# sebrahimi1988/dss-ml-at-scale

Measured on NVIDIA H100. Metric: series fitted+forecast/sec, higher is better.
Workload: dtype f32

## Files before the change

### dss-ml-at-scale_b200/csrc/fit_tc.cu

```cuda
#include "mmf_internal.cuh"
#include "sm90_ptx.cuh"

namespace mmf {
namespace {

using namespace sm90;

constexpr int TILE_M = 128;
constexpr int KC = 32;
constexpr int NGROUPS = 2;
constexpr int FOLD_CHUNKS = 18;
constexpr int MAX_PRED = 64;
constexpr int BULK_MAX_PRED = 28;
constexpr int Y_STAGE_BYTES = TILE_M * KC * 4;
constexpr int AT_STAGE_BYTES = 2 * P * KC * 4;
constexpr int THREADS = 416;
constexpr int TILE_RING = 4;
constexpr int WARP_EPI0 = 8, WARP_PROD = 12;

template <int STAGES, int OBUF, bool SE = false>
struct SmemLayoutT {
  static constexpr int y = 0;
  static constexpr int at = y + STAGES * Y_STAGE_BYTES;
  static constexpr int apred = at + STAGES * AT_STAGE_BYTES;
  static constexpr int ostage = apred + MAX_PRED * P * 4;
  static constexpr int acc = ostage + OBUF * TILE_M * BULK_MAX_PRED * 4;
  static constexpr int nm = acc + 2 * NGROUPS * TILE_M * P * 4;
  static constexpr int cc = nm + 2 * NGROUPS * TILE_M * 2;
  static constexpr int tiles = cc + 2 * TILE_M * 4;
  static constexpr int bars = tiles + TILE_RING * 4;
  static constexpr int n_bars = 2 * STAGES + 6 + 2 * TILE_RING;
  static constexpr int ss = bars + n_bars * 8;
  static constexpr int sfac = ss + (SE ? 2 * NGROUPS * TILE_M * 8 : 0);
  static constexpr int total = sfac + (SE ? MAX_PRED * 4 : 0);
  static_assert(total + 1024 <= 232448, "exceeds the 227 KB of shared memory a CTA can opt into");
};

__device__ __forceinline__ float dot16(const float* __restrict__ arow, const float (&g)[P], float s) {
  const float4* ap = reinterpret_cast<const float4*>(arow);
  const float4 a0 = ap[0], a1 = ap[1], a2 = ap[2], a3 = ap[3];
  s = fmaf(a0.x, g[0], s);  s = fmaf(a0.y, g[1], s);  s = fmaf(a0.z, g[2], s);  s = fmaf(a0.w, g[3], s);
  s = fmaf(a1.x, g[4], s);  s = fmaf(a1.y, g[5], s);  s = fmaf(a1.z, g[6], s);  s = fmaf(a1.w, g[7], s);
  s = fmaf(a2.x, g[8], s);  s = fmaf(a2.y, g[9], s);  s = fmaf(a2.z, g[10], s); s = fmaf(a2.w, g[11], s);
  s = fmaf(a3.x, g[12], s); s = fmaf(a3.y, g[13], s); s = fmaf(a3.z, g[14], s); s = fmaf(a3.w, g[15], s);
  return s;
}

__device__ __forceinline__ bool is_finite_bits(float x) { return (__float_as_uint(x) & 0x7f800000u) != 0x7f800000u; }

__device__ __forceinline__ float centring_constant(const float4& a, const float4& b, int t_fit) {
  const float v[8] = {a.x, a.y, a.z, a.w, b.x, b.y, b.z, b.w};
  float c = t_fit > 7 ? v[7] : __int_as_float(0x7fc00000);
#pragma unroll
  for (int i = 6; i >= 0; --i) c = (i < t_fit && is_finite_bits(v[i])) ? v[i] : c;
  return c;
}

__device__ __forceinline__ void bt_write_moments(const BtArgs& bt, int k, int grp, int64_t n, const TileRec& tr, int frow0,
                                                 int t4, const float (&acc)[2][P], bool folded, const float* sacc) {
#pragma unroll
  for (int h = 0; h < 2; ++h)
#pragma unroll
    for (int j = 0; j < 2; ++j) {
      const int rt = 64 * h + frow0 + 8 * j;
      if (rt >= tr.nrows) continue;
      float* __restrict__ dst = bt.mom + (((int64_t)k * 2 + grp) * n + tr.row0 + rt) * P + 2 * t4;
#pragma unroll
      for (int i = 0; i < 2; ++i) {
        const int q = 4 * i + 2 * j;
        float2 v = make_float2(acc[h][q] + acc[h][q + P / 2], acc[h][q + 1] + acc[h][q + 1 + P / 2]);
        if (folded) {
          const float2 o = *reinterpret_cast<const float2*>(sacc + rt * P + 8 * i + 2 * t4);
          v.x = o.x + v.x; v.y = o.y + v.y;
        }
        *reinterpret_cast<float2*>(dst + 8 * i) = v;
      }
    }
}

__device__ __forceinline__ float lds32(uint32_t addr) {
  float v;
  asm volatile("ld.shared.f32 %0, [%1];" : "=f"(v) : "r"(addr));
  return v;
}

template <int STAGES, int OBUF, bool MULTI, bool SE = false, bool BT = false>
__global__ void __launch_bounds__(THREADS, 1)
fit_tc_kernel(const __grid_constant__ TcLaunch tl, const DesignView d, const FitArgs a,
              uint32_t* __restrict__ pending_count, const int n_tiles, const int n_chunks, const MultiView mv,
              const SeArgs se, const BtArgs bt) {
  static_assert(!SE || !MULTI, "standard errors are built for the single-calendar launch");
  static_assert(!BT || !(MULTI || SE), "backtests are built for the single-calendar launch");
  using SmemLayout = SmemLayoutT<STAGES, OBUF, SE>;
  auto tile_rec = [&](int ti) -> TileRec {
    if (MULTI) {
      if (ti >= n_tiles) return TileRec{0, 0, 0, 1};
      const int4 v = __ldg(reinterpret_cast<const int4*>(mv.tiles) + ti);
      return TileRec{v.x, v.y, v.z, v.w};
    }
    const int64_t left = a.n - (int64_t)ti * TILE_M;
    return TileRec{ti * TILE_M, (int)(left >= TILE_M ? TILE_M : (left > 0 ? left : 0)), 0, n_chunks};
  };
  extern __shared__ unsigned char smem_dyn[];
  unsigned char* smem = reinterpret_cast<unsigned char*>((reinterpret_cast<uintptr_t>(smem_dyn) + 1023) & ~uintptr_t(1023));
  const uint32_t sbase = smem_u32(smem);
  const uint32_t s_y = sbase + SmemLayout::y;
  const uint32_t s_at = sbase + SmemLayout::at;
  float* s_apred = reinterpret_cast<float*>(smem + SmemLayout::apred);
  float* s_ostage = reinterpret_cast<float*>(smem + SmemLayout::ostage);
  float* s_acc = reinterpret_cast<float*>(smem + SmemLayout::acc);
  uint16_t* s_nm = reinterpret_cast<uint16_t*>(smem + SmemLayout::nm);
  float* s_cc = reinterpret_cast<float*>(smem + SmemLayout::cc);
  double* s_ss = reinterpret_cast<double*>(smem + SmemLayout::ss);
  float* s_sfac = reinterpret_cast<float*>(smem + SmemLayout::sfac);
#ifdef MMF_TC_NO_COLLECT
  const bool collect = false;
#else
  const bool collect = a.recs != nullptr && d.t_fit <= 65535;
#endif
  const uint32_t s_bars = sbase + SmemLayout::bars;
  const int warp = threadIdx.x >> 5;
  const int lane = threadIdx.x & 31;
  auto bar_full = [&](int s) { return s_bars + 8u * s; };
  auto bar_empty = [&](int s) { return s_bars + 8u * (STAGES + s); };
  auto bar_accfull = [&](int b) { return s_bars + 8u * (2 * STAGES + b); };
  auto bar_accempty = [&](int b) { return s_bars + 8u * (2 * STAGES + 2 + b); };
  auto bar_cc = [&](int b) { return s_bars + 8u * (2 * STAGES + 4 + b); };
  auto bar_tfull = [&](int s) { return s_bars + 8u * (2 * STAGES + 6 + s); };
  auto bar_tempty = [&](int s) { return s_bars + 8u * (2 * STAGES + 6 + TILE_RING + s); };
  int* s_tiles = reinterpret_cast<int*>(smem + SmemLayout::tiles);
  auto take_tile = [&](int lt) -> int {
    const int sl = lt % TILE_RING;
    mbar_wait(bar_tfull(sl), (lt / TILE_RING) & 1);
    const int t = *reinterpret_cast<volatile int*>(s_tiles + sl);
    __syncwarp();
    if (lane == 0) mbar_arrive(bar_tempty(sl));
    return t;
  };

  if (blockIdx.x == 0 && threadIdx.x == 0 && a.zero_next != nullptr) {
#pragma unroll
    for (int i = 0; i < CTR_WORDS; ++i) a.zero_next[i] = 0u;
  }
  if (warp == WARP_PROD) {
    if (lane == 0) {
      for (int s = 0; s < STAGES; ++s) {
        mbar_init(bar_full(s), 1);
        mbar_init(bar_empty(s), 4);
      }
      for (int b = 0; b < 2; ++b) {
        mbar_init(bar_accfull(b), NGROUPS * 128);
        mbar_init(bar_accempty(b), 4);
        mbar_init(bar_cc(b), 128);
      }
      for (int sl = 0; sl < TILE_RING; ++sl) {
        mbar_init(bar_tfull(sl), 1);
        mbar_init(bar_tempty(sl), NGROUPS * 4 + 4);
      }
      fence_mbar_init();
      prefetch_tensormap(tl.tmap_y);
      prefetch_tensormap(tl.tmap_at);
    }
  } else if (warp >= WARP_EPI0) {
    if (!a.skip_pred && !MULTI)
      for (int i = threadIdx.x - WARP_EPI0 * 32; i < a.n_pred * P; i += 128)
        s_apred[i] = __ldg(d.apred + (size_t)a.pred_start * P + i);
    if (SE && !a.skip_pred)
      for (int i = threadIdx.x - WARP_EPI0 * 32; i < a.n_pred; i += 128) s_sfac[i] = __ldg(se.sfac + a.pred_start + i);
  }
  __syncthreads();
  if (threadIdx.x == 0) pdl_launch_dependents();

  if (warp == WARP_PROD) {
    int stage = 0;
    uint32_t phase = 0;
    int last_cal = -1;
    uint32_t* claim_ctr = pending_count + CTR_TILE_CLAIM;
    int tile = blockIdx.x;
    for (int lt = 0;; ++lt) {
      const int sl = lt % TILE_RING;
      mbar_wait(bar_tempty(sl), ((lt / TILE_RING) & 1) ^ 1u);
      const bool more = tile < n_tiles;
      uint32_t claim = 0;
      if (lane == 0) {
        if (more) claim = atomicAdd(claim_ctr, 1u);
        s_tiles[sl] = more ? tile : -1;
        mbar_arrive(bar_tfull(sl));
      }
      __syncwarp();
      if (!more) break;
      const TileRec tr = tile_rec(tile);
      const void* tmy = MULTI ? static_cast<const void*>(mv.tmaps_y + (size_t)tr.cal * 128) : static_cast<const void*>(tl.tmap_y);
      if (MULTI && tr.cal != last_cal) { fence_tensormap_acquire(tmy); last_cal = tr.cal; }
      const int at_row = MULTI ? tr.cal * 2 * P : 0;
      for (int ch = 0; ch < tr.n_chunks; ++ch) {
        mbar_wait(bar_empty(stage), phase ^ 1u);
        tma_load_2d_x2_elect(bar_full(stage), Y_STAGE_BYTES + AT_STAGE_BYTES,
                             s_y + stage * Y_STAGE_BYTES, tmy, ch * KC, tr.row0, L2_EVICT_NORMAL,
                             s_at + stage * AT_STAGE_BYTES, tl.tmap_at, ch * KC, at_row,
                             MULTI ? L2_EVICT_NORMAL : L2_EVICT_LAST);
        if (++stage == STAGES) { stage = 0; phase ^= 1u; }
      }
      tile = static_cast<int>(gridDim.x + __shfl_sync(0xffffffffu, claim, 0));
    }
  } else if (warp < NGROUPS * 4) {
    const int grp = warp >> 2;
    const int r = threadIdx.x & 127;
    const uint32_t row_off = static_cast<uint32_t>(r) * 128u;
    const uint32_t sw = static_cast<uint32_t>(r & 7);
    const int g8 = lane >> 2, t4 = lane & 3;
    const int frow0 = 16 * (warp & 3) + g8;
    uint32_t gc = 0;
    for (int lt = 0;; ++lt) {
      const int tile = take_tile(lt);
      if (tile < 0) break;
      const TileRec tr = tile_rec(tile);
      bool bad = false;
      float cf[2][2];
      float acc[2][P];
#pragma unroll
      for (int h = 0; h < 2; ++h)
#pragma unroll
        for (int i = 0; i < P; ++i) acc[h][i] = 0.f;
      const bool scan = collect && (!MULTI || r < tr.nrows);
      const int seg = (grp ^ (int)gc) & 1;
      int nm = 0;
      unsigned long long packq = 0ull;
      const int ab = lt & 1;
      float* __restrict__ sacc = s_acc + (ab * NGROUPS + grp) * TILE_M * P;
      auto sacc_at = [&](int h, int j, int i) {
        return reinterpret_cast<float2*>(sacc + (64 * h + frow0 + 8 * j) * P + 8 * i + 2 * t4);
      };
      bool folded = false;
      int since_fold = 0;
      double ssq[2][2] = {{0.0, 0.0}, {0.0, 0.0}};
      for (int ch = seg; ch < tr.n_chunks; ch += NGROUPS) {
        const uint32_t k = gc + static_cast<uint32_t>(ch);
        const int stage = static_cast<int>(k % STAGES);
        mbar_wait(bar_full(stage), (k / STAGES) & 1u);
        const uint32_t sy = s_y + stage * Y_STAGE_BYTES;
        if (ch == seg) {
          if (seg == 0) {
            mbar_wait(bar_accempty(ab), ((lt >> 1) & 1) ^ 1u);
            float c = 0.f;
            if (d.has_constant && r < tr.nrows) {
              const uint32_t rowp = sy + row_off;
              c = centring_constant(lds128(rowp + (sw << 4)), lds128(rowp + ((1u ^ sw) << 4)), MULTI ? KC : d.t_fit);
            }
            bad = collect && !is_finite_bits(c);
            s_cc[ab * TILE_M + r] = bad ? 0.f : c;
            mbar_arrive(bar_cc(ab));
          }
          mbar_wait(bar_cc(ab), (lt >> 1) & 1);
#pragma unroll
          for (int h = 0; h < 2; ++h)
#pragma unroll
            for (int j = 0; j < 2; ++j) cf[h][j] = s_cc[ab * TILE_M + 64 * h + frow0 + 8 * j];
        }
        if (scan) {
          const uint32_t rowp = sy + row_off;
          float4 v[8];
#pragma unroll
          for (int q = 0; q < 8; ++q) v[q] = lds128(rowp + ((static_cast<uint32_t>(q) ^ sw) << 4));
          float chk = 0.f;
#pragma unroll
          for (int q = 0; q < 8; ++q) {
            chk = fmaf(v[q].x, 0.f, chk); chk = fmaf(v[q].y, 0.f, chk);
            chk = fmaf(v[q].z, 0.f, chk); chk = fmaf(v[q].w, 0.f, chk);
          }
          if (!(chk == 0.f)) {
            unsigned gaps = 0u;
#pragma unroll
            for (int q = 0; q < 8; ++q)
              gaps |= (is_finite_bits(v[q].x) ? 0u : 1u << (4 * q)) | (is_finite_bits(v[q].y) ? 0u : 2u << (4 * q)) |
                      (is_finite_bits(v[q].z) ? 0u : 4u << (4 * q)) | (is_finite_bits(v[q].w) ? 0u : 8u << (4 * q));
            uint16_t* __restrict__ mt = a.recs[(int64_t)tr.row0 + r].miss_t + seg * SOLVE_SEG;
            const int tbase = ch * KC;
            while (gaps) {
              const int pos = __ffs(gaps) - 1;
              gaps &= gaps - 1u;
              packq = (packq >> 16) | (static_cast<unsigned long long>(tbase + pos) << 48);
              ++nm;
              if ((nm & 3) == 0 && nm <= SOLVE_SEG) *reinterpret_cast<unsigned long long*>(mt + nm - 4) = packq;
              if constexpr (BT) if (nm == SOLVE_SEG + 1)
                reinterpret_cast<uint16_t*>(&a.recs[(int64_t)tr.row0 + r].ss)[seg] = static_cast<uint16_t>(tbase + pos);
            }
          }
        }
        uint32_t ahi[2][KC / 8][4], alo[2][KC / 8][4];
        const int lim = d.t_fit - ch * KC;
#pragma unroll
        for (int h = 0; h < 2; ++h)
#pragma unroll
          for (int j = 0; j < 2; ++j) {
            const uint32_t rowp = sy + static_cast<uint32_t>(64 * h + frow0 + 8 * j) * 128u + t4 * 4;
            float part = 0.f;
#pragma unroll
            for (int kk = 0; kk < KC / 8; ++kk)
#pragma unroll
              for (int hf = 0; hf < 2; ++hf) {
                float x = lds32(rowp + ((static_cast<uint32_t>(2 * kk + hf) ^ static_cast<uint32_t>(g8)) << 4));
                if (collect) x = is_finite_bits(x) ? x : cf[h][j];
                const float rr = x - cf[h][j];
                const uint32_t hb = __float_as_uint(rr) & 0xFFFFE000u;
                ahi[h][kk][j + 2 * hf] = hb;
                alo[h][kk][j + 2 * hf] = __float_as_uint(rr - __uint_as_float(hb));
                if (SE) {
                  const float rs = 4 * (2 * kk + hf) + t4 < lim ? rr : 0.f;
                  part = fmaf(rs, rs, part);
                }
              }
            if (SE) ssq[h][j] += static_cast<double>(part);
          }
        const uint64_t bdesc0 = gmma_desc_k_sw128(s_at + stage * AT_STAGE_BYTES);
        uint32_t bt_in = 0;
        if constexpr (BT) {
          const int s0 = ch * KC;
          uint32_t pre = 0;
#pragma unroll
          for (int k = 0; k < MMF_BT_MAX_ORIGINS - 1; ++k) {
            pre |= (bt.t_orig[k] >= s0 - KC && bt.t_orig[k] <= s0 ? 1u : 0u) << k;
            bt_in |= (bt.t_orig[k] > s0 && bt.t_orig[k] < s0 + KC ? 1u : 0u) << k;
          }
          while (pre) {
            const int k = __ffs(pre) - 1;
            pre &= pre - 1u;
            bt_write_moments(bt, k, grp, a.n, tr, frow0, t4, acc, folded, sacc);
          }
        }
        if constexpr (BT) {
        if (bt_in != 0u) {
          int lo = 0;
          uint32_t m = bt_in;
          for (;;) {
            const int k = m ? __ffs(m) - 1 : -1;
            const int hi = k >= 0 ? __ldg(&bt.cals[k].t_fit) - ch * KC : KC;
            wgmma_fence();
#pragma unroll
            for (int h = 0; h < 2; ++h)
#pragma unroll
              for (int kk = 0; kk < KC / 8; ++kk) {
                const uint64_t bdesc = bdesc0 + static_cast<uint64_t>(kk * 2);
                uint32_t fh[4], fl[4];
#pragma unroll
                for (int e = 0; e < 4; ++e) {
                  const int col = 8 * kk + 4 * (e >> 1) + t4;
                  const bool in = col >= lo && col < hi;
                  fh[e] = in ? ahi[h][kk][e] : 0u;
                  fl[e] = in ? alo[h][kk][e] : 0u;
                }
                wgmma_m64n32k8_tf32_rs(acc[h], fh, bdesc);
#ifndef MMF_TC_NO_LO_TERM
                wgmma_m64n32k8_tf32_rs(acc[h], fl, bdesc);
#endif
              }
            wgmma_commit();
            wgmma_wait<0>();
            wgmma_fence_regs(acc[0]);
            wgmma_fence_regs(acc[1]);
            if (k < 0) break;
            bt_write_moments(bt, k, grp, a.n, tr, frow0, t4, acc, folded, sacc);
            m &= m - 1u;
            lo = hi;
          }
        } else {
        wgmma_fence();
#pragma unroll
        for (int h = 0; h < 2; ++h)
#pragma unroll
          for (int kk = 0; kk < KC / 8; ++kk) {
            const uint64_t bdesc = bdesc0 + static_cast<uint64_t>(kk * 2);
            wgmma_m64n32k8_tf32_rs(acc[h], ahi[h][kk], bdesc);
#ifndef MMF_TC_NO_LO_TERM
            wgmma_m64n32k8_tf32_rs(acc[h], alo[h][kk], bdesc);
#endif
          }
        wgmma_commit();
        wgmma_wait<0>();
        wgmma_fence_regs(acc[0]);
        wgmma_fence_regs(acc[1]);
        }
        } else {
        wgmma_fence();
#pragma unroll
        for (int h = 0; h < 2; ++h)
#pragma unroll
          for (int kk = 0; kk < KC / 8; ++kk) {
            const uint64_t bdesc = bdesc0 + static_cast<uint64_t>(kk * 2);
            wgmma_m64n32k8_tf32_rs(acc[h], ahi[h][kk], bdesc);
#ifndef MMF_TC_NO_LO_TERM
            wgmma_m64n32k8_tf32_rs(acc[h], alo[h][kk], bdesc);
#endif
          }
        wgmma_commit();
        wgmma_wait<0>();
        wgmma_fence_regs(acc[0]);
        wgmma_fence_regs(acc[1]);
        }
        __syncwarp();
        if (lane == 0) mbar_arrive(bar_empty(stage));
        if (++since_fold == FOLD_CHUNKS && ch + NGROUPS < tr.n_chunks) {
          if (!folded) mbar_wait(bar_accempty(ab), ((lt >> 1) & 1) ^ 1u);
#pragma unroll
          for (int h = 0; h < 2; ++h)
#pragma unroll
            for (int j = 0; j < 2; ++j)
#pragma unroll
              for (int i = 0; i < 2; ++i) {
                const int q = 4 * i + 2 * j;
                float2 f = make_float2(acc[h][q] + acc[h][q + P / 2], acc[h][q + 1] + acc[h][q + 1 + P / 2]);
                if (folded) { const float2 o = *sacc_at(h, j, i); f.x = o.x + f.x; f.y = o.y + f.y; }
                *sacc_at(h, j, i) = f;
              }
#pragma unroll
          for (int h = 0; h < 2; ++h)
#pragma unroll
            for (int i = 0; i < P; ++i) acc[h][i] = 0.f;
          folded = true;
          since_fold = 0;
        }
      }
      if (scan && (nm & 3) != 0 && nm < SOLVE_SEG) {
        uint16_t* __restrict__ mt = a.recs[(int64_t)tr.row0 + r].miss_t + seg * SOLVE_SEG;
        *reinterpret_cast<unsigned long long*>(mt + (nm & ~3)) = packq >> (16 * (4 - (nm & 3)));
      }
      if constexpr (BT) {
        const int s_end = ((tr.n_chunks - 1 - seg) / NGROUPS * NGROUPS + seg + 1) * KC;
        uint32_t rest = 0;
#pragma unroll
        for (int k = 0; k < MMF_BT_MAX_ORIGINS - 1; ++k) rest |= (bt.t_orig[k] != INT32_MAX && bt.t_orig[k] >= s_end ? 1u : 0u) << k;
        while (rest) {
          const int k = __ffs(rest) - 1;
          rest &= rest - 1u;
          bt_write_moments(bt, k, grp, a.n, tr, frow0, t4, acc, folded, sacc);
        }
      }
      if (!folded) mbar_wait(bar_accempty(ab), ((lt >> 1) & 1) ^ 1u);
#pragma unroll
      for (int h = 0; h < 2; ++h)
#pragma unroll
        for (int j = 0; j < 2; ++j)
#pragma unroll
          for (int i = 0; i < 2; ++i) {
            const int q = 4 * i + 2 * j;
            float2 v = make_float2(acc[h][q] + acc[h][q + P / 2], acc[h][q + 1] + acc[h][q + 1 + P / 2]);
            if (folded) { const float2 o = *sacc_at(h, j, i); v.x = o.x + v.x; v.y = o.y + v.y; }
            *sacc_at(h, j, i) = v;
          }
      if (SE) {
#pragma unroll
        for (int h = 0; h < 2; ++h)
#pragma unroll
          for (int j = 0; j < 2; ++j) {
            double v = ssq[h][j];
            v += __shfl_xor_sync(0xffffffffu, v, 1);
            v += __shfl_xor_sync(0xffffffffu, v, 2);
            if (t4 == 0) s_ss[(ab * NGROUPS + grp) * TILE_M + 64 * h + frow0 + 8 * j] = v;
          }
      }
      const int cnt = nm > 0x7ffe ? 0x7ffe : nm;
      s_nm[(ab * NGROUPS + seg) * TILE_M + r] = static_cast<uint16_t>(cnt | (bad ? 0x8000 : 0));
      mbar_arrive(bar_accfull(ab));
      gc += static_cast<uint32_t>(tr.n_chunks);
    }
  } else {
    const int r = threadIdx.x & 127;
    bool vec_out = (a.n_pred % 4 == 0) && (a.ld_out % 4 == 0) && ((reinterpret_cast<uintptr_t>(a.out) & 15u) == 0);
    for (int i = 0; i + 1 < a.n_out; ++i) vec_out = vec_out && ((reinterpret_cast<uintptr_t>(a.out_more[i]) & 15u) == 0);
#ifdef MMF_TC_NO_BULK
    const bool bulk = false;
#else
    const bool bulk = !a.skip_pred && vec_out && a.out_multimem != 1 && a.ld_out == a.n_pred && a.n_pred <= BULK_MAX_PRED;
#endif
    const uint32_t s_ostage_u32 = smem_u32(s_ostage);
    const uint64_t l2_policy = l2_evict_first_policy();
    const bool se_vec = SE && (a.n_pred % 4 == 0) && (se.ld_se % 4 == 0) &&
                        ((reinterpret_cast<uintptr_t>(se.out_se) & 15u) == 0);
    int lt = 0;
    int cur_cal = MULTI ? -1 : 0;
    uint32_t kept_mask = d.kept_mask;
    int t_fit_c = d.t_fit;
    for (;; ++lt) {
      const int tile = take_tile(lt);
      if (tile < 0) break;
      const int ab = lt & 1;
      const TileRec tr = tile_rec(tile);
      const int64_t row = (int64_t)tr.row0 + r;
      const bool live = r < tr.nrows;
      if (MULTI && tr.cal != cur_cal) {
        const int4* cp = reinterpret_cast<const int4*>(mv.cals + tr.cal);
        const int4 m0 = __ldg(cp), m1 = __ldg(cp + 1);
        t_fit_c = m0.x;
        kept_mask = static_cast<uint32_t>(m0.w);
        if (!a.skip_pred) {
          named_bar_sync(2, 128);
          const float* __restrict__ src = d.apred + (size_t)(m1.x + m1.y) * P;
          for (int i = threadIdx.x - WARP_EPI0 * 32; i < a.n_pred * P; i += 128) s_apred[i] = __ldg(src + i);
          named_bar_sync(2, 128);
        }
        cur_cal = tr.cal;
      }
      mbar_wait(bar_accfull(ab), (lt >> 1) & 1);
      float c = s_cc[ab * TILE_M + r];
      float g[P];
      {
        const float4* p0 = reinterpret_cast<const float4*>(s_acc + (ab * NGROUPS + 0) * TILE_M * P + r * P);
        const float4* p1 = reinterpret_cast<const float4*>(s_acc + (ab * NGROUPS + 1) * TILE_M * P + r * P);
#pragma unroll
        for (int q = 0; q < P / 4; ++q) {
          const float4 u = p0[q], w = p1[q];
          g[4 * q] = u.x + w.x; g[4 * q + 1] = u.y + w.y; g[4 * q + 2] = u.z + w.z; g[4 * q + 3] = u.w + w.w;
        }
      }
      const unsigned f0 = s_nm[(ab * NGROUPS + 0) * TILE_M + r], f1 = s_nm[(ab * NGROUPS + 1) * TILE_M + r];
      const double ss = SE ? s_ss[(ab * NGROUPS + 0) * TILE_M + r] + s_ss[(ab * NGROUPS + 1) * TILE_M + r] : 0.0;
      if constexpr (BT) {
        __syncwarp();
        if (lane == 0) mbar_arrive(bar_accempty(ab));
        for (int k = 0; k < bt.n_origin; ++k) {
          const bool last = k == bt.n_origin - 1;
          const int4 m0 = __ldg(reinterpret_cast<const int4*>(bt.cals + k));
          const int tk = m0.x;
          float gk[P];
          if (last || !live) {
#pragma unroll
            for (int p = 0; p < P; ++p) gk[p] = g[p];
          } else {
            const float4* p0 = reinterpret_cast<const float4*>(bt.mom + (((int64_t)k * NGROUPS + 0) * a.n + row) * P);
            const float4* p1 = reinterpret_cast<const float4*>(bt.mom + (((int64_t)k * NGROUPS + 1) * a.n + row) * P);
#pragma unroll
            for (int q = 0; q < P / 4; ++q) {
              const float4 u = p0[q], w = p1[q];
              gk[4 * q] = u.x + w.x; gk[4 * q + 1] = u.y + w.y; gk[4 * q + 2] = u.z + w.z; gk[4 * q + 3] = u.w + w.w;
            }
          }
          const SolveRec* __restrict__ src = collect ? a.recs + row : nullptr;
          int n0 = f0 & 0x7fff, n1 = f1 & 0x7fff;
          bool over = false;
          if (collect && !last && live && (n0 | n1) != 0) {
#pragma unroll
            for (int sg = 0; sg < 2; ++sg) {
              const int tot = sg ? n1 : n0;
              const uint16_t* mt = src->miss_t + sg * SOLVE_SEG;
              const int have = tot < SOLVE_SEG ? tot : SOLVE_SEG;
              int cnt = 0;
              while (cnt < have && mt[cnt] < tk) ++cnt;
              if (cnt == SOLVE_SEG && tot > SOLVE_SEG && reinterpret_cast<const uint16_t*>(&src->ss)[sg] < tk) over = true;
              if (sg) n1 = cnt; else n0 = cnt;
            }
          }
          bool general = false;
          if (collect)
            general = ((f0 | f1) & 0x8000u) != 0u || over || n0 > SOLVE_SEG || n1 > SOLVE_SEG || 2 * (n0 + n1) > tk;
          bool finite = true;
#pragma unroll
          for (int p = 0; p < P; ++p) {
            finite = finite && is_finite_bits(gk[p]);
            if (!((kept_mask >> p) & 1u)) gk[p] = 0.f;
          }
          const bool pend = live && (!finite || general);
          const bool defer = live && !pend && (n0 + n1) > 0;
          const unsigned pm = __ballot_sync(0xffffffffu, pend);
          if (lane == 0 && pm != 0u) {
            atomicAdd(pending_count, __popc(pm));
            atomicAdd(bt.pending + k, __popc(pm));
          }
          const unsigned dm = __ballot_sync(0xffffffffu, defer);
          if (dm != 0u) {
            unsigned base = 0;
            if (lane == 0) base = atomicAdd(bt.rec_count + k, __popc(dm));
            base = __shfl_sync(0xffffffffu, base, 0);
            if (defer) {
              SolveRec& rec = bt.recs[(int64_t)k * a.n + row];
              float bk[P];
              if (last) {
#pragma unroll
                for (int p = 0; p < P; ++p) bk[p] = gk[p];
              } else {
                const float* __restrict__ tm = bt.tmat + (size_t)k * P * P;
#pragma unroll
                for (int p = 0; p < P; ++p) {
                  float s = 0.f;
#pragma unroll
                  for (int q = 0; q < P; ++q) s = fmaf(__ldg(tm + q * P + p), gk[q], s);
                  bk[p] = s;
                }
                for (int sg = 0; sg < 2; ++sg) {
                  const int cnt = sg ? n1 : n0;
                  for (int e = 0; e < cnt; ++e) rec.miss_t[sg * SOLVE_SEG + e] = src->miss_t[sg * SOLVE_SEG + e];
                }
              }
              float4* bp = reinterpret_cast<float4*>(rec.b);
              bp[0] = make_float4(bk[0], bk[1], bk[2], bk[3]);    bp[1] = make_float4(bk[4], bk[5], bk[6], bk[7]);
              bp[2] = make_float4(bk[8], bk[9], bk[10], bk[11]);  bp[3] = make_float4(bk[12], bk[13], bk[14], bk[15]);
              rec.c = c;
              rec.nm[0] = static_cast<uint16_t>(n0);
              rec.nm[1] = static_cast<uint16_t>(n1);
              rec.cal = k;
              const unsigned slot = base + __popc(dm & ((1u << lane) - 1u));
              if (slot < a.rec_cap) bt.rec_rows[(int64_t)k * a.n + slot] = row;
            }
          }
          if (live && !pend && !defer) {
            const float* __restrict__ pk = bt.pred + (size_t)k * a.n_pred * P;
            const int64_t off = ((int64_t)k * bt.out_kstride + row) * a.ld_out;
            if (vec_out) {
              for (int j = 0; j < a.n_pred; j += 4) {
                float o[4];
#pragma unroll
                for (int w = 0; w < 4; ++w) o[w] = dot16(pk + (j + w) * P, gk, c);
                store_out4(a, off + j, make_float4(o[0], o[1], o[2], o[3]));
              }
            } else {
              for (int j = 0; j < a.n_pred; ++j) store_out1(a, off + j, dot16(pk + j * P, gk, c));
            }
          }
          if (live) a.status[(int64_t)k * bt.st_kstride + row] = pend ? MMF_STATUS_PENDING : (defer ? MMF_STATUS_DEFERRED : MMF_STATUS_OK);
        }
        continue;
      }
      __syncwarp();
      if (lane == 0) mbar_arrive(bar_accempty(ab));
      int nm0 = 0, nm1 = 0;
      bool general = false;
      if (collect) {
        nm0 = f0 & 0x7fff; nm1 = f1 & 0x7fff;
        general = ((f0 | f1) & 0x8000u) != 0u || nm0 > SOLVE_SEG || nm1 > SOLVE_SEG || 2 * (nm0 + nm1) > t_fit_c;
        if (general) c = 0.f;
      }
      bool finite = true;
#pragma unroll
      for (int p = 0; p < P; ++p) {
        finite = finite && is_finite_bits(g[p]);
        if (!((kept_mask >> p) & 1u)) g[p] = 0.f;
      }
      const bool pend = live && (!finite || general);
      const bool defer = live && !pend && (nm0 + nm1) > 0;
      const unsigned pm = __ballot_sync(0xffffffffu, pend);
      if (lane == 0 && pm != 0u) {
        atomicAdd(pending_count, __popc(pm));
        if (MULTI) atomicAdd(mv.pending_by_cal + tr.cal, __popc(pm));
      }
      const unsigned dm = __ballot_sync(0xffffffffu, defer);
      if (dm != 0u) {
        unsigned base = 0;
        if (lane == 0) base = atomicAdd(a.rec_count, __popc(dm));
        base = __shfl_sync(0xffffffffu, base, 0);
        if (defer) {
          SolveRec& rec = a.recs[row];
          float4* bp = reinterpret_cast<float4*>(rec.b);
          bp[0] = make_float4(g[0], g[1], g[2], g[3]);    bp[1] = make_float4(g[4], g[5], g[6], g[7]);
          bp[2] = make_float4(g[8], g[9], g[10], g[11]);  bp[3] = make_float4(g[12], g[13], g[14], g[15]);
          rec.c = c;
          if (SE) rec.ss = static_cast<float>(ss);
          rec.nm[0] = static_cast<uint16_t>(nm0);
          rec.nm[1] = static_cast<uint16_t>(nm1);
          rec.cal = tr.cal;
          const unsigned slot = base + __popc(dm & ((1u << lane) - 1u));
          if (slot < a.rec_cap) a.rec_rows[slot] = row;
        }
      }
      if (bulk) {
        const int ob = OBUF > 1 ? (lt % OBUF) : 0;
        if (warp == WARP_EPI0) { if (OBUF > 1) bulk_wait_read1_elect(); else bulk_wait_read_elect(); }
        named_bar_sync(1, 128);
        float* __restrict__ srow = s_ostage + ob * (TILE_M * BULK_MAX_PRED) + r * a.n_pred;
        for (int k = 0; k < a.n_pred; k += 4) {
          float o[4];
#pragma unroll
          for (int w = 0; w < 4; ++w) o[w] = dot16(s_apred + (k + w) * P, g, c);
          *reinterpret_cast<float4*>(srow + k) = make_float4(o[0], o[1], o[2], o[3]);
        }
        fence_proxy_async_smem();
        named_bar_sync(1, 128);
        const uint32_t bytes = static_cast<uint32_t>(tr.nrows) * a.n_pred * 4u;
        const int64_t off = (int64_t)tr.row0 * a.n_pred;
        const uint32_t src = s_ostage_u32 + static_cast<uint32_t>(ob) * (TILE_M * BULK_MAX_PRED * 4);
        for (uint32_t i = r; i < bytes / 16u; i += 128u)
          stg128_hint(reinterpret_cast<float4*>(a.out + off) + i, lds128(src + 16u * i), l2_policy);
        if (warp == WARP_EPI0) {
          const int n_peer = a.n_out - 1;
          int j = n_peer > 1 ? tile % n_peer : 0;
          for (int i = 0; i < n_peer; ++i) {
            bulk_store_elect(reinterpret_cast<uint64_t>(a.out_more[j] + off), src, bytes);
            if (++j == n_peer) j = 0;
          }
          bulk_commit_elect();
        }
      } else if (live && !pend && !defer && !a.skip_pred) {
        const int64_t off = row * a.ld_out;
        if (vec_out) {
          for (int k = 0; k < a.n_pred; k += 4) {
            float o[4];
#pragma unroll
            for (int w = 0; w < 4; ++w) o[w] = dot16(s_apred + (k + w) * P, g, c);
            store_out4(a, off + k, make_float4(o[0], o[1], o[2], o[3]));
          }
        } else {
          for (int k = 0; k < a.n_pred; ++k) store_out1(a, off + k, dot16(s_apred + k * P, g, c));
        }
      }
      if (live) {
        if (!pend && !defer) {
          if (a.out_gamma != nullptr) {
            float4* gp = reinterpret_cast<float4*>(a.out_gamma + row * P);
            gp[0] = make_float4(g[0], g[1], g[2], g[3]);    gp[1] = make_float4(g[4], g[5], g[6], g[7]);
            gp[2] = make_float4(g[8], g[9], g[10], g[11]);  gp[3] = make_float4(g[12], g[13], g[14], g[15]);
            a.out_c[row] = c;
          }
          if (a.out_beta != nullptr) {
            float* __restrict__ br = a.out_beta + row * P;
            for (int p = 0; p < P; ++p) {
              float s = (p == 0 && d.has_constant) ? c : 0.f;
#pragma unroll
              for (int q = 0; q < P; ++q) s = fmaf(__ldg(d.w + p * P + q), g[q], s);
              br[p] = s;
            }
          }
          if (SE) {
            double bg = 0.0;
#pragma unroll
            for (int p = 0; p < P; ++p) bg = fma(static_cast<double>(g[p]), static_cast<double>(g[p]), bg);
            const int dof = t_fit_c - __popc(kept_mask);
            const double rss = fmax(ss - bg, 0.0);
            const float sig = dof > 0 ? static_cast<float>(sqrt(rss / dof)) : __int_as_float(0x7fc00000);
            se.sigma[row] = sig;
            if (se.dof != nullptr) se.dof[row] = dof;
            if (se.out_se != nullptr && !a.skip_pred) {
              float* __restrict__ srow = se.out_se + row * se.ld_se;
              int k = 0;
              if (se_vec)
                for (; k < a.n_pred; k += 4)
                  __stcs(reinterpret_cast<float4*>(srow + k),
                         make_float4(sig * s_sfac[k], sig * s_sfac[k + 1], sig * s_sfac[k + 2], sig * s_sfac[k + 3]));
              for (; k < a.n_pred; ++k) __stcs(srow + k, sig * s_sfac[k]);
            }
          }
        }
        stg32_hint(a.status + row, pend ? MMF_STATUS_PENDING : (defer ? MMF_STATUS_DEFERRED : MMF_STATUS_OK), l2_policy);
      }
    }
    if (bulk && warp == WARP_EPI0) bulk_wait_all_elect();
  }
}

}

bool fit_tc_supported(const DesignView& d, const FitArgs& a, const char** why) {
  const char* w = nullptr;
  if (!a.skip_pred && a.n_pred > MAX_PRED) w = "n_pred > 64 needs the fit + predict_tc_kernel pair";
  else if (a.n_pred < 1) w = "n_pred < 1";
  else if (a.ld_y % 4 != 0) w = "ld_y not a multiple of 4 floats (TMA needs 16-B row pitch)";
  else if ((reinterpret_cast<uintptr_t>(a.y) & 15u) != 0) w = "y not 16-B aligned";
  else if (d.t_fit < 1) w = "t_fit < 1";
  else if (a.n > (int64_t)0x7fffffff - TILE_M) w = "n too large for 32-bit TMA coordinates";
  if (why) *why = w;
  return w == nullptr;
}

template <int STAGES, int OBUF, bool MULTI, bool SE = false, bool BT = false>
static cudaError_t launch_variant(const DesignView& d, const FitArgs& a, const TcLaunch& tl, uint32_t* pending_count,
                                  int sm_count, cudaStream_t s, int n_tiles, int n_chunks, const MultiView& mv,
                                  const SeArgs& se = SeArgs{}, const BtArgs& bt = BtArgs{}) {
  const size_t smem = SmemLayoutT<STAGES, OBUF, SE>::total + 1024;
  cudaError_t e = cudaFuncSetAttribute(fit_tc_kernel<STAGES, OBUF, MULTI, SE, BT>, cudaFuncAttributeMaxDynamicSharedMemorySize, (int)smem);
  if (e != cudaSuccess) return e;
  const int grid = n_tiles < sm_count ? n_tiles : sm_count;
  fit_tc_kernel<STAGES, OBUF, MULTI, SE, BT><<<grid, THREADS, smem, s>>>(tl, d, a, pending_count, n_tiles, n_chunks, mv, se, bt);
  return cudaGetLastError();
}

cudaError_t launch_fit_tc(const DesignView& d, const FitArgs& a, const TcLaunch& tl, uint32_t* pending_count,
                          int sm_count, cudaStream_t s, int variant, const MultiView* multi) {
  if (a.n <= 0) return cudaSuccess;
  if (multi != nullptr)
    return launch_variant<8, 1, true>(d, a, tl, pending_count, sm_count, s, multi->n_tiles, 2, *multi);
  const int n_tiles = (int)((a.n + TILE_M - 1) / TILE_M);
  const int n_chunks = d.t_pad / KC;
  const MultiView none{};
  return variant == 2 ? launch_variant<6, 2, false>(d, a, tl, pending_count, sm_count, s, n_tiles, n_chunks, none)
                      : launch_variant<8, 1, false>(d, a, tl, pending_count, sm_count, s, n_tiles, n_chunks, none);
}

cudaError_t launch_fit_tc_se(const DesignView& d, const FitArgs& a, const TcLaunch& tl, uint32_t* pending_count,
                             int sm_count, cudaStream_t s, const SeArgs& se) {
  if (a.n <= 0) return cudaSuccess;
  const int n_tiles = (int)((a.n + TILE_M - 1) / TILE_M);
  return launch_variant<8, 1, false, true>(d, a, tl, pending_count, sm_count, s, n_tiles, d.t_pad / KC, MultiView{}, se);
}

cudaError_t launch_fit_tc_bt(const DesignView& d, const FitArgs& a, const TcLaunch& tl, uint32_t* pending_count,
                             int sm_count, cudaStream_t s, const BtArgs& bt) {
  if (a.n <= 0) return cudaSuccess;
  const int n_tiles = (int)((a.n + TILE_M - 1) / TILE_M);
  return launch_variant<8, 1, false, false, true>(d, a, tl, pending_count, sm_count, s, n_tiles, d.t_pad / KC,
                                                  MultiView{}, SeArgs{}, bt);
}

}
```

Before: 634.9 million.

## Batch forecast output writes across several staged tiles before flushing

```diff
diff --git a/dss-ml-at-scale_b200/csrc/fit_tc.cu b/dss-ml-at-scale_b200/csrc/fit_tc.cu
--- a/dss-ml-at-scale_b200/csrc/fit_tc.cu
+++ b/dss-ml-at-scale_b200/csrc/fit_tc.cu
@@ -32,7 +32,8 @@
   static constexpr int n_bars = 2 * STAGES + 6 + 2 * TILE_RING;
   static constexpr int ss = bars + n_bars * 8;
   static constexpr int sfac = ss + (SE ? 2 * NGROUPS * TILE_M * 8 : 0);
-  static constexpr int total = sfac + (SE ? MAX_PRED * 4 : 0);
+  static constexpr int otiles = sfac + (SE ? MAX_PRED * 4 : 0);
+  static constexpr int total = otiles + (OBUF > 1 ? OBUF * 4 : 0);
   static_assert(total + 1024 <= 232448, "exceeds the 227 KB of shared memory a CTA can opt into");
 };
 
@@ -91,6 +92,7 @@
               const SeArgs se, const BtArgs bt) {
   static_assert(!SE || !MULTI, "standard errors are built for the single-calendar launch");
   static_assert(!BT || !(MULTI || SE), "backtests are built for the single-calendar launch");
+  static_assert(STAGES % 2 == 0, "each stage must belong to one consumer group");
   using SmemLayout = SmemLayoutT<STAGES, OBUF, SE>;
   auto tile_rec = [&](int ti) -> TileRec {
     if (MULTI) {
@@ -476,6 +478,20 @@
     const uint64_t l2_policy = l2_evict_first_policy();
     const bool se_vec = SE && (a.n_pred % 4 == 0) && (se.ld_se % 4 == 0) &&
                         ((reinterpret_cast<uintptr_t>(se.out_se) & 15u) == 0);
+    int ns = 0;
+    int* s_otiles = reinterpret_cast<int*>(smem + SmemLayout::otiles);
+    const int epoch = OBUF * static_cast<int>(gridDim.x);
+    int next_flush = epoch;
+    auto flush_staged = [&]() {
+      for (int b = 0; b < ns; ++b) {
+        const TileRec tb = tile_rec(s_otiles[b]);
+        const uint32_t bytes = static_cast<uint32_t>(tb.nrows) * a.n_pred * 4u;
+        float4* __restrict__ dst = reinterpret_cast<float4*>(a.out + (int64_t)tb.row0 * a.n_pred);
+        const uint32_t src = s_ostage_u32 + static_cast<uint32_t>(b) * (TILE_M * BULK_MAX_PRED * 4);
+        for (uint32_t i = r; i < bytes / 16u; i += 128u) stg128_hint(dst + i, lds128(src + 16u * i), l2_policy);
+      }
+      ns = 0;
+    };
     int lt = 0;
     int cur_cal = MULTI ? -1 : 0;
     uint32_t kept_mask = d.kept_mask;
@@ -661,8 +677,8 @@
         }
       }
       if (bulk) {
-        const int ob = OBUF > 1 ? (lt % OBUF) : 0;
-        if (warp == WARP_EPI0) { if (OBUF > 1) bulk_wait_read1_elect(); else bulk_wait_read_elect(); }
+        const int ob = OBUF > 1 ? ns : 0;
+        if (warp == WARP_EPI0 && ob == 0) bulk_wait_read_elect();
         named_bar_sync(1, 128);
         float* __restrict__ srow = s_ostage + ob * (TILE_M * BULK_MAX_PRED) + r * a.n_pred;
         for (int k = 0; k < a.n_pred; k += 4) {
@@ -671,13 +687,15 @@
           for (int w = 0; w < 4; ++w) o[w] = dot16(s_apred + (k + w) * P, g, c);
           *reinterpret_cast<float4*>(srow + k) = make_float4(o[0], o[1], o[2], o[3]);
         }
+        if (OBUF > 1 && r == 0) s_otiles[ob] = tile;
         fence_proxy_async_smem();
         named_bar_sync(1, 128);
         const uint32_t bytes = static_cast<uint32_t>(tr.nrows) * a.n_pred * 4u;
         const int64_t off = (int64_t)tr.row0 * a.n_pred;
         const uint32_t src = s_ostage_u32 + static_cast<uint32_t>(ob) * (TILE_M * BULK_MAX_PRED * 4);
-        for (uint32_t i = r; i < bytes / 16u; i += 128u)
-          stg128_hint(reinterpret_cast<float4*>(a.out + off) + i, lds128(src + 16u * i), l2_policy);
+        if constexpr (OBUF == 1)
+          for (uint32_t i = r; i < bytes / 16u; i += 128u)
+            stg128_hint(reinterpret_cast<float4*>(a.out + off) + i, lds128(src + 16u * i), l2_policy);
         if (warp == WARP_EPI0) {
           const int n_peer = a.n_out - 1;
           int j = n_peer > 1 ? tile % n_peer : 0;
@@ -686,6 +704,13 @@
             if (++j == n_peer) j = 0;
           }
           bulk_commit_elect();
+        }
+        if constexpr (OBUF > 1) {
+          ++ns;
+          if (ns == OBUF || tile >= next_flush) {
+            flush_staged();
+            next_flush = (tile / epoch + 1) * epoch;
+          }
         }
       } else if (live && !pend && !defer && !a.skip_pred) {
         const int64_t off = row * a.ld_out;
@@ -740,6 +765,7 @@
         stg32_hint(a.status + row, pend ? MMF_STATUS_PENDING : (defer ? MMF_STATUS_DEFERRED : MMF_STATUS_OK), l2_policy);
       }
     }
+    if constexpr (OBUF > 1) if (bulk && ns > 0) flush_staged();
     if (bulk && warp == WARP_EPI0) bulk_wait_all_elect();
   }
 }
@@ -777,9 +803,8 @@
     return launch_variant<8, 1, true>(d, a, tl, pending_count, sm_count, s, multi->n_tiles, 2, *multi);
   const int n_tiles = (int)((a.n + TILE_M - 1) / TILE_M);
   const int n_chunks = d.t_pad / KC;
-  const MultiView none{};
-  return variant == 2 ? launch_variant<6, 2, false>(d, a, tl, pending_count, sm_count, s, n_tiles, n_chunks, none)
-                      : launch_variant<8, 1, false>(d, a, tl, pending_count, sm_count, s, n_tiles, n_chunks, none);
+  (void)variant;
+  return launch_variant<6, 4, false>(d, a, tl, pending_count, sm_count, s, n_tiles, n_chunks, MultiView{});
 }
 
 cudaError_t launch_fit_tc_se(const DesignView& d, const FitArgs& a, const TcLaunch& tl, uint32_t* pending_count,
```

New measurement: 650.6 million (median of 6 runs). 1.02x the previous value.
